# DRL-Navigation/DDRL4NAV

Hardware: AMD Instinct MI355X
Metric: env-steps/sec (whole node) + PPO update ms, Pong 256 envs at 1/2/4/8 GPUs (higher is better)
Workload: dtype f32 (f16x3 MFMA planes, fp32 accumulate)

## Files before the change

### ddrl4nav_amd/csrc/conv2.hip

```cpp
#include "engine2.h"

namespace ddrl {


using u4v = __attribute__((ext_vector_type(4))) unsigned;

constexpr int F1_PITCH = 168;
template <int NE>
struct Fwd1B {
  static constexpr int ROWS = 32 * NE, A_BYTES = 4 * NPL * 2 * ROWS * 16, PITCH = F1_PITCH, IMG_BYTES = 64 * PITCH;
  static constexpr int STAGE_BYTES = A_BYTES + IMG_BYTES, AQ = A_BYTES / 16, NAJ = AQ / 256;
  static constexpr size_t LDS_BYTES = 2 * STAGE_BYTES;
};

template <int NE, bool IND = false>
__global__ __launch_bounds__(256) void conv_fwd1_planes_kernel(const uint8_t* __restrict__ frames, const unsigned short* __restrict__ wp1b,
                                                               float* __restrict__ amax, const float* __restrict__ params, int64_t bias_off0,
                                                               int64_t bias_off1, float* __restrict__ out, int64_t out_es, int n,
                                                               unsigned* __restrict__ m1, int64_t m1_es, int C,
                                                               const int32_t* __restrict__ tab, int64_t n_planes) {
  using K = Fwd1B<NE>;
  extern __shared__ __attribute__((aligned(16))) char ldsb[];
  const int tid = threadIdx.x, lane = tid & 63, wc = tid >> 6, l31 = lane & 31, hi = lane >> 5;
  const int c0 = blockIdx.x * 256, ctot = n * C1_P, clast = min(c0 + 255, ctot - 1);
  const int b0 = c0 / 400, b1 = clast / 400, oyf0 = (c0 % 400) / 20, iy0_start = 4 * oyf0;
  int nrows0, nrows1 = 0;
  if (b1 == b0) {
    nrows0 = 4 * ((clast % 400) / 20 - oyf0) + 8;
  } else {
    nrows0 = 84 - iy0_start;
    nrows1 = 4 * ((clast % 400) / 20) + 8;
  }
  const int nd0 = nrows0 * 21, nd_total = nd0 + nrows1 * 21;
  const int64_t src0 = (int64_t)b0 * (C * 7056) + iy0_start * 84, src1 = (int64_t)b1 * (C * 7056);
  if (blockIdx.x == 0 && tid < (AMAX_DH - AMAX_FIRST_ACT) * 2) amax[amax_idx(AMAX_FIRST_ACT, 0) + tid] = 0.0f;
  int64_t imsrc[6];
  int imdst[6];
  int imoff[6];
  unsigned imsel = 0u;
#pragma unroll
  for (int j = 0; j < 6; ++j) {
    const int idx = tid + 256 * j;
    if constexpr (IND) {
      const bool second = idx < nd_total && idx >= nd0;
      imoff[j] = second ? (idx - nd0) * 4 : iy0_start * 84 + (idx < nd0 ? idx * 4 : 0);
      imsel |= (second ? 1u : 0u) << j;
    } else {
      imsrc[j] = (idx >= nd_total) ? src0 : (idx < nd0 ? src0 + idx * 4 : src1 + (idx - nd0) * 4);
    }
    imdst[j] = K::A_BYTES + (idx / 21) * K::PITCH + (idx % 21) * 8;
  }
  int abase[NE], bbase[2];
#pragma unroll
  for (int i = 0; i < NE; ++i) abase[i] = (hi * K::ROWS + i * 32 + l31) * 16;
#pragma unroll
  for (int j = 0; j < 2; ++j) {
    int c = c0 + wc * 64 + j * 32 + l31;
    if (c >= ctot) c = c0;
    const int b = c / 400, pix = c % 400, oy = pix / 20, ox = pix % 20;
    const int lr = (b == b0) ? (4 * oy - iy0_start) : (nrows0 + 4 * oy);
    bbase[j] = K::A_BYTES + (lr + hi) * K::PITCH + ox * 8;
  }
  unsigned imreg[4][6];
  if constexpr (IND) {
#pragma unroll
    for (int ch = 0; ch < 4; ++ch) {
      const int64_t pb0 = frame_plane_base(tab, b0, ch, n_planes), pb1 = frame_plane_base(tab, b1, ch, n_planes);
#pragma unroll
      for (int j = 0; j < 6; ++j) imreg[ch][j] = *(const unsigned*)(frames + (((imsel >> j) & 1u) ? pb1 : pb0) + imoff[j]);
    }
  } else {
#pragma unroll
    for (int ch = 0; ch < 4; ++ch)
#pragma unroll
      for (int j = 0; j < 6; ++j) imreg[ch][j] = *(const unsigned*)(frames + (ch < C ? ch : C - 1) * 7056 + imsrc[j]);
  }
  const int wave = wave_u();
  uint32_t woff[K::NAJ];
#pragma unroll
  for (int j = 0; j < K::NAJ; ++j) woff[j] = (uint32_t)((tid + 256 * j) * 16);
  auto stage_w = [&](int ch, char* st) {
    direct_copy((const char*)wp1b + (size_t)ch * K::A_BYTES, woff, (float*)st, wave, tid, K::AQ);
  };
  auto commit_img = [&](char* st, int ch) {
#pragma unroll
    for (int j = 0; j < 6; ++j) {
      if (tid + 256 * j < nd_total) {
        const unsigned v = imreg[ch][j];
        *(uint2*)(st + imdst[j]) = pixel_quad(v);
      }
    }
  };
  f32x16 acc[NE][2];
#pragma unroll
  for (int i = 0; i < NE; ++i)
#pragma unroll
    for (int j = 0; j < 2; ++j)
#pragma unroll
      for (int r = 0; r < 16; ++r) acc[i][j][r] = 0.0f;
  stage_w(0, ldsb);
  commit_img(ldsb, 0);
  wait_vmcnt<0>();
  __syncthreads();
#pragma unroll
  for (int ch = 0; ch < 4; ++ch) {
    if (ch >= C) break;
    const char* cur = ldsb + (ch & 1) * K::STAGE_BYTES;
    char* nxt = ldsb + ((ch + 1) & 1) * K::STAGE_BYTES;
    if (ch + 1 < C) stage_w(ch + 1, nxt);
#pragma unroll
    for (int g = 0; g < 4; ++g) {
      frag8 b[2];
#pragma unroll
      for (int j = 0; j < 2; ++j) {
        const uint2 lo = *(const uint2*)(cur + bbase[j] + g * (2 * K::PITCH));
        const uint2 hi4 = *(const uint2*)(cur + bbase[j] + g * (2 * K::PITCH) + 8);
        b[j] = __builtin_bit_cast(frag8, (u4v){lo.x, lo.y, hi4.x, hi4.y});
      }
#pragma unroll
      for (int p = NPL - 1; p >= 0; --p) {
        frag8 a[NE];
#pragma unroll
        for (int i = 0; i < NE; ++i) a[i] = *(const frag8*)(cur + abase[i] + ((g * NPL + p) * 2) * K::ROWS * 16);
#pragma unroll
        for (int i = 0; i < NE; ++i)
#pragma unroll
          for (int j = 0; j < 2; ++j) acc[i][j] = mfma_planes(a[i], b[j], acc[i][j]);
      }
    }
    if (ch + 1 < C) {
      commit_img(nxt, ch + 1);
      wait_vmcnt<0>();
    }
    __syncthreads();
  }
  float* bias = (float*)ldsb;
  if (tid < K::ROWS) bias[tid] = params[(tid >> 5 ? bias_off1 : bias_off0) + (tid & 31)];
  __syncthreads();
  float r255[NE];
#pragma unroll
  for (int i = 0; i < NE; ++i) r255[i] = 1.0f / (255.0f * plane_scale(amax[amax_idx(AMAX_W1, i)]));
#pragma unroll
  for (int j = 0; j < 2; ++j) {
    const int c = c0 + wc * 64 + j * 32 + l31;
    if (c >= ctot) continue;
    const int b = c / 400, pix = c % 400;
    const uint32_t lanep = (uint32_t)((b * A1_N + pix + hi * (4 * C1_P)) * 4);
#pragma unroll
    for (int i = 0; i < NE; ++i) {
      float* base = out + i * out_es;
      unsigned bits = 0u;
#pragma unroll
      for (int r = 0; r < 16; ++r) {
        const int oc = acc_row(r, hi);
        const float y = leaky_f(__builtin_fmaf(acc[i][j][r], r255[i], bias[i * 32 + oc]));
        st1_so(base + acc_row(r, 0) * C1_P, lanep, y);
        bits = __builtin_amdgcn_alignbit(bits, (unsigned)__builtin_elementwise_sub_sat((int)__float_as_uint(y), 1), 31);
      }
      if (m1 != nullptr) ((unsigned short*)(m1 + i * m1_es))[2 * (int64_t)c + hi] = (unsigned short)bits;
    }
  }
}

template <int NE>
struct Fwd1R {
  static constexpr int ROWS = 32 * NE, A_BYTES = 4 * NPL * 2 * ROWS * 16, PITCH = F1_PITCH, IMG_BYTES = 64 * PITCH;
  static constexpr int W_BYTES = 4 * A_BYTES, IMG_OFF = W_BYTES, GROUP_IMG = 4 * IMG_BYTES;
  static constexpr int BIAS_OFF = IMG_OFF + 2 * GROUP_IMG;
  static constexpr size_t LDS_BYTES = BIAS_OFF + ROWS * 4;
  static_assert(LDS_BYTES <= 160 * 1024, "one workgroup per CU");
};

template <int NE, bool IND = false>
__global__ __launch_bounds__(512) void conv_fwd1_resident_kernel(const uint8_t* __restrict__ frames, const unsigned short* __restrict__ wp1b,
                                                                 float* __restrict__ amax, const float* __restrict__ params, int64_t bias_off0,
                                                                 int64_t bias_off1, float* __restrict__ out, int64_t out_es, int n,
                                                                 unsigned* __restrict__ m1, int64_t m1_es, int C,
                                                                 const int32_t* __restrict__ tab, int64_t n_planes) {
  using K = Fwd1R<NE>;
  extern __shared__ __attribute__((aligned(16))) char ldsr[];
  const int tid = threadIdx.x, gq = tid >> 8, lt = tid & 255, lane = tid & 63, wc = (tid >> 6) & 3, l31 = lane & 31, hi = lane >> 5;
  char* img = ldsr + K::IMG_OFF + gq * K::GROUP_IMG;
  float* bias = (float*)(ldsr + K::BIAS_OFF);
  const int ctot = n * C1_P, ntiles = (ctot + 255) / 256;
  if (blockIdx.x == 0 && tid < (AMAX_DH - AMAX_FIRST_ACT) * 2) amax[amax_idx(AMAX_FIRST_ACT, 0) + tid] = 0.0f;
  for (int q = tid; q < C * (K::A_BYTES / 16); q += 512) *(f4*)(ldsr + q * 16) = *(const f4*)((const char*)wp1b + (size_t)q * 16);
  if (tid < K::ROWS) bias[tid] = params[(tid >> 5 ? bias_off1 : bias_off0) + (tid & 31)];
  float r255[NE];
#pragma unroll
  for (int i = 0; i < NE; ++i) r255[i] = 1.0f / (255.0f * plane_scale(amax[amax_idx(AMAX_W1, i)]));
  int abase[NE];
#pragma unroll
  for (int i = 0; i < NE; ++i) abase[i] = (hi * K::ROWS + i * 32 + l31) * 16;

  struct Geo {
    int c0, b0, iy0_start, nrows0, nd0, nd_total;
    int64_t src0, src1;
    int64_t pb[2][4];
  };
  auto geometry = [&](int t) {
    Geo g;
    g.c0 = t * 256;
    const int clast = min(g.c0 + 255, ctot - 1);
    g.b0 = g.c0 / 400;
    const int b1 = clast / 400, oyf0 = (g.c0 % 400) / 20;
    g.iy0_start = 4 * oyf0;
    int nrows1 = 0;
    if (b1 == g.b0) {
      g.nrows0 = 4 * ((clast % 400) / 20 - oyf0) + 8;
    } else {
      g.nrows0 = 84 - g.iy0_start;
      nrows1 = 4 * ((clast % 400) / 20) + 8;
    }
    g.nd0 = g.nrows0 * 21;
    g.nd_total = g.nd0 + nrows1 * 21;
    if constexpr (IND) {
      const int ub0 = __builtin_amdgcn_readfirstlane(g.b0), ub1 = __builtin_amdgcn_readfirstlane(b1);
#pragma unroll
      for (int ch = 0; ch < 4; ++ch) {
        g.pb[0][ch] = frame_plane_base(tab, ub0, ch, n_planes);
        g.pb[1][ch] = frame_plane_base(tab, ub1, ch, n_planes);
      }
      return g;
    }
    g.src0 = (int64_t)g.b0 * (C * 7056) + g.iy0_start * 84;
    g.src1 = (int64_t)b1 * (C * 7056);
    return g;
  };
  unsigned imreg[4][6];
  auto request = [&](const Geo& g) {
#pragma unroll
    for (int j = 0; j < 6; ++j) {
      const int idx = lt + 256 * j;
      if constexpr (IND) {
        const bool second = idx < g.nd_total && idx >= g.nd0;
        const int o = second ? (idx - g.nd0) * 4 : g.iy0_start * 84 + (idx < g.nd0 ? idx * 4 : 0);
#pragma unroll
        for (int ch = 0; ch < 4; ++ch) {
          const int64_t p0 = g.pb[0][ch], p1 = g.pb[1][ch];
          imreg[ch][j] = *(const unsigned*)(frames + (second ? p1 : p0) + o);
        }
        continue;
      }
      const int64_t o = (idx >= g.nd_total) ? g.src0 : (idx < g.nd0 ? g.src0 + idx * 4 : g.src1 + (idx - g.nd0) * 4);
#pragma unroll
      for (int ch = 0; ch < 4; ++ch) imreg[ch][j] = *(const unsigned*)(frames + (ch < C ? ch : C - 1) * 7056 + o);
    }
  };
  int t = 2 * (int)blockIdx.x + gq;
  Geo g = geometry(min(t, ntiles - 1));
  request(g);
  __syncthreads();
  for (; 2 * (t / 2) < ntiles; t += 2 * (int)gridDim.x) {
    const bool live = t < ntiles;
#pragma unroll
    for (int ch = 0; ch < 4; ++ch)
#pragma unroll
      for (int j = 0; j < 6; ++j) {
        const int idx = lt + 256 * j;
        if (ch < C && idx < g.nd_total) *(uint2*)(img + ch * K::IMG_BYTES + (idx / 21) * K::PITCH + (idx % 21) * 8) = pixel_quad(imreg[ch][j]);
      }
    int bbase[2];
#pragma unroll
    for (int j = 0; j < 2; ++j) {
      int c = g.c0 + wc * 64 + j * 32 + l31;
      if (c >= ctot) c = g.c0;
      const int b = c / 400, pix = c % 400, oy = pix / 20, ox = pix % 20;
      const int lr = (b == g.b0) ? (4 * oy - g.iy0_start) : (g.nrows0 + 4 * oy);
      bbase[j] = (lr + hi) * K::PITCH + ox * 8;
    }
    const Geo cur = g;
    __syncthreads();
    const int tn = t + 2 * (int)gridDim.x;
    if (2 * (tn / 2) < ntiles) {
      g = geometry(min(tn, ntiles - 1));
      request(g);
    }
    f32x16 acc[NE][2];
#pragma unroll
    for (int i = 0; i < NE; ++i)
#pragma unroll
      for (int j = 0; j < 2; ++j)
#pragma unroll
        for (int r = 0; r < 16; ++r) acc[i][j][r] = 0.0f;
#pragma unroll
    for (int ch = 0; ch < 4; ++ch) {
      if (ch >= C) break;
#pragma unroll
      for (int gk = 0; gk < 4; ++gk) {
        frag8 b[2];
#pragma unroll
        for (int j = 0; j < 2; ++j) {
          const char* q = img + ch * K::IMG_BYTES + bbase[j] + gk * (2 * K::PITCH);
          const uint2 lo = *(const uint2*)q, hi4 = *(const uint2*)(q + 8);
          b[j] = __builtin_bit_cast(frag8, (u4v){lo.x, lo.y, hi4.x, hi4.y});
        }
#pragma unroll
        for (int p = NPL - 1; p >= 0; --p) {
          frag8 a[NE];
#pragma unroll
          for (int i = 0; i < NE; ++i) a[i] = *(const frag8*)(ldsr + ch * K::A_BYTES + abase[i] + ((gk * NPL + p) * 2) * K::ROWS * 16);
#pragma unroll
          for (int i = 0; i < NE; ++i)
#pragma unroll
            for (int j = 0; j < 2; ++j) acc[i][j] = mfma_planes(a[i], b[j], acc[i][j]);
        }
      }
    }
    __syncthreads();
    if (!live) continue;
#pragma unroll
    for (int j = 0; j < 2; ++j) {
      const int c = cur.c0 + wc * 64 + j * 32 + l31;
      if (c >= ctot) continue;
      const int b = c / 400, pix = c % 400;
      const uint32_t lanep = (uint32_t)((b * A1_N + pix + hi * (4 * C1_P)) * 4);
#pragma unroll
      for (int i = 0; i < NE; ++i) {
        float* base = out + i * out_es;
        unsigned bits = 0u;
#pragma unroll
        for (int r = 0; r < 16; ++r) {
          const int oc = acc_row(r, hi);
          const float y = leaky_f(__builtin_fmaf(acc[i][j][r], r255[i], bias[i * 32 + oc]));
          st1_so(base + acc_row(r, 0) * C1_P, lanep, y);
          bits = __builtin_amdgcn_alignbit(bits, (unsigned)__builtin_elementwise_sub_sat((int)__float_as_uint(y), 1), 31);
        }
        if (m1 != nullptr) ((unsigned short*)(m1 + i * m1_es))[2 * (int64_t)c + hi] = (unsigned short)bits;
      }
    }
  }
}

template <int NE, bool IND>
static void launch_fwd1_planes(const EncCall& c, bool acting, hipStream_t st) {
  const Workspace& w = *c.ws;
  const ParamLayout& L = *c.L;
  if (!acting && (int64_t)c.n * C1_P >= 256 * 2048) {
    using R = Fwd1R<NE>;
    lds_limit_once<conv_fwd1_resident_kernel<NE, IND>>((int)R::LDS_BYTES);
    static const int cus = [] {
      int dev = 0;
      hipDeviceProp_t prop;
      return hipGetDevice(&dev) == hipSuccess && hipGetDeviceProperties(&prop, dev) == hipSuccess ? prop.multiProcessorCount : 256;
    }();
    hipLaunchKernelGGL((conv_fwd1_resident_kernel<NE, IND>), dim3((unsigned)cus), dim3(512), R::LDS_BYTES, st, c.frames, w.wp1b, w.amax, c.params,
                       L.enc_base[0] + L.enc.c1b, L.enc_base[NE - 1] + L.enc.c1b, w.a1, w.es(A1_N), c.n, w.m1, w.es(M1_N), L.C, c.tab, c.n_planes);
    return;
  }
  using K = Fwd1B<NE>;
  lds_limit_once<conv_fwd1_planes_kernel<NE, IND>>((int)K::LDS_BYTES);
  hipLaunchKernelGGL((conv_fwd1_planes_kernel<NE, IND>), dim3((unsigned)(((int64_t)c.n * C1_P + 255) / 256)), dim3(256), K::LDS_BYTES, st, c.frames,
                     w.wp1b, w.amax, c.params, L.enc_base[0] + L.enc.c1b, L.enc_base[NE - 1] + L.enc.c1b, w.a1, w.es(A1_N), c.n,
                     acting ? (unsigned*)nullptr : w.m1, w.es(M1_N), L.C, c.tab, c.n_planes);
}
template <int NE>
static void launch_fwd1(const EncCall& c, bool acting, hipStream_t st) {
  if (c.tab != nullptr) {
    launch_fwd1_planes<NE, true>(c, acting, st);
  } else {
    launch_fwd1_planes<NE, false>(c, acting, st);
  }
}

struct Fwd2B {
  static constexpr int SPT = 3, KC = 2;
  static constexpr int WPE = 3;
  static constexpr int ROW = 52, CH = 20 * ROW, IMG_PLANE = SPT * KC * CH;
  static constexpr int W_OFF = NPL * IMG_PLANE, W_BYTES = KC * NPL * 64 * 32;
  static constexpr int BIAS_OFF = W_OFF + W_BYTES;
  static constexpr int NIU = SPT * KC * 100, NIJ = (NIU + 255) / 256;
  static constexpr int NWJ = W_BYTES / 16 / 256;
  static constexpr int STAGE_BYTES = BIAS_OFF;
  static constexpr size_t LDS_BYTES = STAGE_BYTES + 64 * 4;
};
struct __attribute__((packed, aligned(4))) lds_u2 {
  unsigned x, y;
};

__global__ __launch_bounds__(256) __attribute__((amdgpu_waves_per_eu(Fwd2B::WPE, Fwd2B::WPE))) void conv_fwd2_planes_kernel(const float* __restrict__ a1, int64_t a1_es, const unsigned short* __restrict__ wp2b,
                                                               float* __restrict__ amax, const float* __restrict__ params, int64_t bias_off0,
                                                               int64_t bias_off1, float* __restrict__ out, int64_t out_es, int n,
                                                               unsigned* __restrict__ m2) {
  using K = Fwd2B;
  extern __shared__ __attribute__((aligned(16))) char ldsc2[];
  const int tid = threadIdx.x, lane = tid & 63, wc = tid >> 6, l31 = lane & 31, hi = lane >> 5;
  const int e = blockIdx.z, b0 = blockIdx.x * K::SPT;
  const float sa = plane_scale(amax[amax_idx(AMAX_A1, e)]), inv = 1.0f / (sa * plane_scale(amax[amax_idx(AMAX_W2, e)]));
  if (tid < 64) ((float*)(ldsc2 + K::STAGE_BYTES))[tid] = params[(e ? bias_off1 : bias_off0) + tid];
  const float* isrc[K::NIJ];
  int idst[K::NIJ];
#pragma unroll
  for (int j = 0; j < K::NIJ; ++j) {
    const int u = min(tid + 256 * j, K::NIU - 1);
    const int s = u / (100 * K::KC), rem = u % (100 * K::KC), q = rem % 100;
    isrc[j] = a1 + e * a1_es + (int64_t)min(b0 + s, n - 1) * A1_N + rem * 4;
    idst[j] = (s * K::KC + rem / 100) * K::CH + (q / 5) * K::ROW + (q % 5) * 8;
  }
  const unsigned short* wsrc = wp2b + (int64_t)e * (32 * NPL * 64 * 16) + tid * 8;
  int aA[2], bB[2];
#pragma unroll
  for (int i = 0; i < 2; ++i) aA[i] = K::W_OFF + (i * 32 + l31) * 32 + hi * 16;
#pragma unroll
  for (int j = 0; j < 2; ++j) {
    int c = wc * 64 + j * 32 + l31;
    if (c >= K::SPT * 81) c = 0;
    const int s = c / 81, pix = c % 81, oy = pix / 9, ox = pix % 9;
    bB[j] = s * K::KC * K::CH + (2 * oy + 2 * hi) * K::ROW + 4 * ox;
  }
  f4 ir[K::NIJ], wr[K::NWJ];
  auto fetch = [&](int kb) {
#pragma unroll
    for (int j = 0; j < K::NIJ; ++j) ir[j] = ld4(isrc[j] + kb * (C1_P * K::KC));
#pragma unroll
    for (int j = 0; j < K::NWJ; ++j) wr[j] = *(const f4*)(wsrc + kb * (K::KC * NPL * 1024) + j * 2048);
  };
  auto commit = [&](char* ldsc2) {
#pragma unroll
    for (int j = 0; j < K::NIJ; ++j) {
      if (j + 1 < K::NIJ || tid + 256 * j < K::NIU) {
        const f4 v = ir[j];
        unsigned pa[NPL], pb[NPL];
        split_planes(v.x, v.y, sa, pa);
        split_planes(v.z, v.w, sa, pb);
        char* d = ldsc2 + idst[j];
#pragma unroll
        for (int p = 0; p < NPL; ++p) *(lds_u2*)(d + p * K::IMG_PLANE) = lds_u2{pa[p], pb[p]};
      }
    }
#pragma unroll
    for (int j = 0; j < K::NWJ; ++j) *(f4*)(ldsc2 + K::W_OFF + (tid + 256 * j) * 16) = wr[j];
  };
  f32x16 acc[2][2];
#pragma unroll
  for (int i = 0; i < 2; ++i)
#pragma unroll
    for (int j = 0; j < 2; ++j)
#pragma unroll
      for (int r = 0; r < 16; ++r) acc[i][j][r] = 0.0f;
  constexpr int NKB = 32 / K::KC;
  auto compute = [&](const char* ldsc2) {
#pragma unroll
    for (int kg = 0; kg < K::KC; ++kg) {
      frag8 a[NPL][2], b[NPL][2];
#pragma unroll
      for (int p = 0; p < NPL; ++p) {
#pragma unroll
        for (int i = 0; i < 2; ++i) a[p][i] = *(const frag8*)(ldsc2 + aA[i] + (kg * NPL + p) * 2048);
#pragma unroll
        for (int j = 0; j < 2; ++j) {
          const char* q = ldsc2 + bB[j] + p * K::IMG_PLANE + kg * K::CH;
          const lds_u2 lo = *(const lds_u2*)q, up = *(const lds_u2*)(q + K::ROW);
          b[p][j] = __builtin_bit_cast(frag8, (u4v){lo.x, lo.y, up.x, up.y});
        }
      }
#pragma unroll
      for (int t = 0; t < NPROD; ++t)
#pragma unroll
        for (int i = 0; i < 2; ++i)
#pragma unroll
          for (int j = 0; j < 2; ++j) acc[i][j] = mfma_planes(a[PA[t]][i], b[PB[t]][j], acc[i][j]);
    }
  };
  fetch(0);
  commit(ldsc2);
  fetch(1);
  __syncthreads();
  for (int kb = 0; kb < NKB; ++kb) {
    compute(ldsc2);
    __syncthreads();
    if (kb + 1 < NKB) {
      commit(ldsc2);
      if (kb + 2 < NKB) fetch(kb + 2);
    }
    __syncthreads();
  }
  const float* bias = (const float*)(ldsc2 + K::STAGE_BYTES);
  float big = 0.0f;
#pragma unroll
  for (int j = 0; j < 2; ++j) {
    const int c = wc * 64 + j * 32 + l31;
    const int s = c / 81, pix = c % 81;
    if (c >= K::SPT * 81 || b0 + s >= n) continue;
    float* base = out + e * out_es + (int64_t)b0 * A2_N;
    const uint32_t lb = (uint32_t)((s * A2_N + pix + hi * (4 * C2_P)) * 4);
    unsigned bits = 0u;
#pragma unroll
    for (int i = 0; i < 2; ++i)
#pragma unroll
      for (int r = 0; r < 16; ++r) {
        const int oc = i * 32 + acc_row(r, hi);
        const float y = leaky_f(__builtin_fmaf(acc[i][j][r], inv, bias[oc]));
        st1_so(base + (i * 32 + acc_row(r, 0)) * C2_P, lb, y);
        big = fmaxf(big, fabsf(y));
        bits = __builtin_amdgcn_alignbit(bits, (unsigned)__builtin_elementwise_sub_sat((int)__float_as_uint(y), 1), 31);
      }
    if (m2 != nullptr) m2[(e * (out_es / A2_N) + b0 + s) * M2_N + pix * 2 + hi] = (bits >> 16) | (bits << 16);
  }
  amax_update(big, amax + amax_idx(AMAX_A2, e));
}
static void launch_fwd2_planes(const EncCall& c, bool acting, hipStream_t st) {
  using K = Fwd2B;
  const Workspace& w = *c.ws;
  const ParamLayout& L = *c.L;
  lds_limit_once<conv_fwd2_planes_kernel>((int)K::LDS_BYTES);
  hipLaunchKernelGGL(conv_fwd2_planes_kernel, dim3((unsigned)((c.n + K::SPT - 1) / K::SPT), 1, (unsigned)L.NE), dim3(256), K::LDS_BYTES, st, w.a1,
                     w.es(A1_N), w.wp2b, w.amax, c.params, L.enc_base[0] + L.enc.c2b, L.enc_base[L.NE - 1] + L.enc.c2b, w.a2, w.es(A2_N),
                     c.n, acting ? (unsigned*)nullptr : w.m2);
}

struct Fwd3B {
  static constexpr int WPE = 3;
  static constexpr int TN = 2, SPT = (128 * TN) / 49, NPX = SPT * 81;
  static constexpr int IMG_PLANE = NPX * 16;
  static constexpr int W_OFF = NPL * IMG_PLANE, W_BYTES = 5 * NPL * 64 * 32;
  static constexpr int BIAS_OFF = W_OFF + W_BYTES;
  static constexpr int NIJ = (NPX + 255) / 256;
  static constexpr int NWJ = (W_BYTES / 16 + 255) / 256;
  static constexpr size_t LDS_BYTES = BIAS_OFF + 64 * 4;
};

__global__ __launch_bounds__(256) __attribute__((amdgpu_waves_per_eu(Fwd3B::WPE, Fwd3B::WPE))) void conv_fwd3_planes_kernel(const float* __restrict__ a2, int64_t a2_es, const unsigned short* __restrict__ wp3b,
                                                               float* __restrict__ amax, const float* __restrict__ params, int64_t bias_off0,
                                                               int64_t bias_off1, float* __restrict__ out, int64_t out_es, int n,
                                                               unsigned* __restrict__ m3) {
  using K = Fwd3B;
  extern __shared__ __attribute__((aligned(16))) char ldsc3[];
  const int tid = threadIdx.x, lane = tid & 63, wc = tid >> 6, l31 = lane & 31, hi = lane >> 5;
  const int e = blockIdx.z, b0 = blockIdx.x * K::SPT;
  const float sa = plane_scale(amax[amax_idx(AMAX_A2, e)]), inv = 1.0f / (sa * plane_scale(amax[amax_idx(AMAX_W3, e)]));
  if (tid < 64) ((float*)(ldsc3 + K::BIAS_OFF))[tid] = params[(e ? bias_off1 : bias_off0) + tid];
  const float* isrc[K::NIJ];
#pragma unroll
  for (int j = 0; j < K::NIJ; ++j) {
    const int u = min(tid + 256 * j, K::NPX - 1);
    const int s = u / 81, px = u % 81;
    isrc[j] = a2 + e * a2_es + (int64_t)min(b0 + s, n - 1) * A2_N + px;
  }
  const unsigned short* wsrc = wp3b + (int64_t)e * (8 * 5 * NPL * 64 * 16) + tid * 8;
  int aA[2], bB[K::TN], tapoff[5];
#pragma unroll
  for (int i = 0; i < 2; ++i) aA[i] = K::W_OFF + (i * 32 + l31) * 32 + hi * 16;
#pragma unroll
  for (int j = 0; j < K::TN; ++j) {
    int c = wc * (32 * K::TN) + j * 32 + l31;
    if (c >= K::SPT * 49) c = 0;
    const int s = c / 49, pix = c % 49;
    bB[j] = (s * 81 + (pix / 7) * 9 + pix % 7) * 16;
  }
#pragma unroll
  for (int kg = 0; kg < 5; ++kg) {
    const int tap = min(2 * kg + hi, 8);
    tapoff[kg] = ((tap / 3) * 9 + tap % 3) * 16;
  }
  float ir[K::NIJ][8];
  f4 wr[K::NWJ];
  auto fetch = [&](int kb) {
#pragma unroll
    for (int j = 0; j < K::NIJ; ++j)
#pragma unroll
      for (int c = 0; c < 8; ++c) ir[j][c] = isrc[j][(kb * 8 + c) * C2_P];
#pragma unroll
    for (int j = 0; j < K::NWJ; ++j)
      if (j + 1 < K::NWJ || tid + 256 * j < K::W_BYTES / 16) wr[j] = *(const f4*)(wsrc + kb * (5 * NPL * 1024) + j * 2048);
  };
  auto commit = [&]() {
#pragma unroll
    for (int j = 0; j < K::NIJ; ++j) {
      if (j + 1 < K::NIJ || tid + 256 * j < K::NPX) {
        unsigned pl[4][NPL];
#pragma unroll
        for (int c = 0; c < 4; ++c) split_planes(ir[j][2 * c], ir[j][2 * c + 1], sa, pl[c]);
        char* d = ldsc3 + (tid + 256 * j) * 16;
#pragma unroll
        for (int p = 0; p < NPL; ++p) *(u4v*)(d + p * K::IMG_PLANE) = (u4v){pl[0][p], pl[1][p], pl[2][p], pl[3][p]};
      }
    }
#pragma unroll
    for (int j = 0; j < K::NWJ; ++j)
      if (j + 1 < K::NWJ || tid + 256 * j < K::W_BYTES / 16) *(f4*)(ldsc3 + K::W_OFF + (tid + 256 * j) * 16) = wr[j];
  };
  f32x16 acc[2][K::TN];
#pragma unroll
  for (int i = 0; i < 2; ++i)
#pragma unroll
    for (int j = 0; j < K::TN; ++j)
#pragma unroll
      for (int r = 0; r < 16; ++r) acc[i][j][r] = 0.0f;
  constexpr int NKB = 8;
  fetch(0);
  commit();
  fetch(1);
  __syncthreads();
  for (int kb = 0; kb < NKB; ++kb) {
#pragma unroll
    for (int kg = 0; kg < 5; ++kg) {
      frag8 a[NPL][2], b[NPL][K::TN];
#pragma unroll
      for (int p = 0; p < NPL; ++p) {
#pragma unroll
        for (int i = 0; i < 2; ++i) a[p][i] = *(const frag8*)(ldsc3 + aA[i] + (kg * NPL + p) * 2048);
#pragma unroll
        for (int j = 0; j < K::TN; ++j) b[p][j] = *(const frag8*)(ldsc3 + bB[j] + tapoff[kg] + p * K::IMG_PLANE);
      }
#pragma unroll
      for (int t = 0; t < NPROD; ++t)
#pragma unroll
        for (int i = 0; i < 2; ++i)
#pragma unroll
          for (int j = 0; j < K::TN; ++j) acc[i][j] = mfma_planes(a[PA[t]][i], b[PB[t]][j], acc[i][j]);
    }
    __syncthreads();
    if (kb + 1 < NKB) {
      commit();
      if (kb + 2 < NKB) fetch(kb + 2);
    }
    __syncthreads();
  }
  const float* bias = (const float*)(ldsc3 + K::BIAS_OFF);
  float big = 0.0f;
#pragma unroll
  for (int j = 0; j < K::TN; ++j) {
    const int c = wc * (32 * K::TN) + j * 32 + l31;
    const int s = c / 49, pix = c % 49;
    if (c >= K::SPT * 49 || b0 + s >= n) continue;
    float* base = out + e * out_es + (int64_t)b0 * FLAT;
    const uint32_t lb = (uint32_t)((s * A3_N + pix + hi * (4 * C3_P)) * 4);
    unsigned bits = 0u;
#pragma unroll
    for (int i = 0; i < 2; ++i)
#pragma unroll
      for (int r = 0; r < 16; ++r) {
        const int oc = i * 32 + acc_row(r, hi);
        const float y = leaky_f(__builtin_fmaf(acc[i][j][r], inv, bias[oc]));
        st1_so(base + (i * 32 + acc_row(r, 0)) * C3_P, lb, y);
        big = fmaxf(big, fabsf(y));
        bits = __builtin_amdgcn_alignbit(bits, (unsigned)__builtin_elementwise_sub_sat((int)__float_as_uint(y), 1), 31);
      }
    if (m3 != nullptr) m3[(e * (out_es / A3_N) + b0 + s) * M3_N + pix * 2 + hi] = (bits >> 16) | (bits << 16);
  }
  amax_update(big, amax + amax_idx(AMAX_A3, e));
}
static void launch_fwd3_planes(const EncCall& c, bool acting, hipStream_t st) {
  using K = Fwd3B;
  const Workspace& w = *c.ws;
  const ParamLayout& L = *c.L;
  lds_limit_once<conv_fwd3_planes_kernel>((int)K::LDS_BYTES);
  hipLaunchKernelGGL(conv_fwd3_planes_kernel, dim3((unsigned)((c.n + K::SPT - 1) / K::SPT), 1, (unsigned)L.NE), dim3(256), K::LDS_BYTES, st, w.a2,
                     w.es(A2_N), w.wp3b, w.amax, c.params, L.enc_base[0] + L.enc.c3b, L.enc_base[L.NE - 1] + L.enc.c3b, w.a3, w.es(A3_N),
                     c.n, acting ? (unsigned*)nullptr : w.m3);
}


void launch_conv_forward(const EncCall& c, bool acting, hipStream_t st) {
  {
    ProfRange pr(c.prof, acting ? "ConvFwd1.act" : "ConvFwd1", st);
    if (c.L->NE == 2) {
      launch_fwd1<2>(c, acting, st);
    } else {
      launch_fwd1<1>(c, acting, st);
    }
  }
  {
    ProfRange pr(c.prof, acting ? "ConvFwd2.act" : "ConvFwd2", st);
    launch_fwd2_planes(c, acting, st);
  }
  {
    ProfRange pr(c.prof, acting ? "ConvFwd3.act" : "ConvFwd3", st);
    launch_fwd3_planes(c, acting, st);
  }
}

struct Dgrad3Rows {
  static constexpr int SPT = 3, NCOL = SPT * 81, NT = 8, ROWW = SPT * 9;
  static constexpr int col_y(int c) { return c / ROWW; }
  static constexpr int col_s(int c) { return c % ROWW / 9; }
  static constexpr int col_x(int c) { return c % 9; }
  static constexpr int tile_y0(int t) { return col_y(32 * t); }
  static constexpr int tile_y1(int t) { return col_y(32 * t + 31 < NCOL ? 32 * t + 31 : NCOL - 1); }
  static constexpr bool tile_has_tap(int t, int tap) { return tap / 3 <= tile_y1(t) && tap / 3 + 6 >= tile_y0(t); }
  static constexpr int tile_taps(int t) {
    int m = 0;
    for (int tap = 0; tap < 9; ++tap) m |= (int)tile_has_tap(t, tap) << tap;
    return m;
  }
  static constexpr int WT = 3, NU = 4;
  static constexpr int WAVE_TILE[4][WT] = {{0, 1, -1}, {5, 6, -1}, {2, 3, 7}, {4, 3, 7}};
  static constexpr int UNIT_I[4][NU] = {{0, 1, 0, 1}, {0, 1, 0, 1}, {0, 1, 0, 0}, {0, 1, 1, 1}};
  static constexpr int UNIT_J[4][NU] = {{0, 0, 1, 1}, {0, 0, 1, 1}, {0, 0, 1, 2}, {0, 0, 1, 2}};
  static constexpr int unit_tile(int w, int u) { return WAVE_TILE[w][UNIT_J[w][u]]; }
  static constexpr int popcount9(int m) {
    int c = 0;
    for (int b = 0; b < 9; ++b) c += m >> b & 1;
    return c;
  }

  static constexpr bool tap_feeds_tile(int t, int tap) {
    for (int c = 32 * t; c < 32 * t + 32 && c < NCOL; ++c) {
      const int sy = col_y(c) - tap / 3, sx = col_x(c) - tap % 3;
      if (sy >= 0 && sy <= 6 && sx >= 0 && sx <= 6) return true;
    }
    return false;
  }
  static constexpr bool masks_are_exact() {
    for (int t = 0; t < NT; ++t)
      for (int tap = 0; tap < 9; ++tap)
        if (tap_feeds_tile(t, tap) != tile_has_tap(t, tap)) return false;
    return true;
  }
  static constexpr bool columns_are_a_permutation() {
    bool seen[NCOL] = {};
    for (int c = 0; c < NCOL; ++c) {
      const int k = col_s(c) * 81 + col_y(c) * 9 + col_x(c);
      if (col_s(c) >= SPT || col_y(c) >= 9 || seen[k]) return false;
      seen[k] = true;
    }
    return true;
  }
  static constexpr int owners(int i, int t) {
    int n = 0;
    for (int w = 0; w < 4; ++w)
      for (int u = 0; u < NU; ++u) n += UNIT_I[w][u] == i && UNIT_J[w][u] < WT && unit_tile(w, u) == t;
    return n;
  }
  static constexpr bool every_unit_has_one_owner() {
    for (int i = 0; i < 2; ++i)
      for (int t = 0; t < NT; ++t)
        if (owners(i, t) != 1) return false;
    return true;
  }
  static constexpr int wave_unit_taps(int w) {
    int n = 0;
    for (int u = 0; u < NU; ++u) n += popcount9(tile_taps(unit_tile(w, u)));
    return n;
  }
  static constexpr int row_tile_taps() {
    int n = 0;
    for (int t = 0; t < NT; ++t) n += popcount9(tile_taps(t));
    return n;
  }
};
static_assert(Dgrad3Rows::NT * 32 >= Dgrad3Rows::NCOL && (Dgrad3Rows::NT - 1) * 32 < Dgrad3Rows::NCOL, "8 column tiles of 32");
static_assert(Dgrad3Rows::columns_are_a_permutation(), "every (sample, pixel) is one column");
static_assert(Dgrad3Rows::masks_are_exact(), "a skipped (tile, tap) reads only the zero border, an issued one reads a dz3 pixel");
static_assert(Dgrad3Rows::every_unit_has_one_owner(), "each of the 16 accumulator tiles belongs to exactly one wave (four each)");
static_assert(Dgrad3Rows::row_tile_taps() == 60, "60 of 72 (column tile, tap) products per row tile");
static_assert(Dgrad3Rows::wave_unit_taps(0) == 30 && Dgrad3Rows::wave_unit_taps(1) == 30 && Dgrad3Rows::wave_unit_taps(2) == 30 &&
                  Dgrad3Rows::wave_unit_taps(3) == 30, "the waves are level: 30 unit-taps = 90 MFMAs per k-block each");

template <int V>
struct RoleC {
  static constexpr int value = V;
};
template <class F>
__device__ __forceinline__ void by_wave_role(int w, F&& f) {
  switch (w) {
    case 0: f(RoleC<0>{}); break;
    case 1: f(RoleC<1>{}); break;
    case 2: f(RoleC<2>{}); break;
    default: f(RoleC<3>{}); break;
  }
}

struct Dgrad3B {
  using R = Dgrad3Rows;
  static constexpr int THREADS = 256, SPT = R::SPT;
  static constexpr int KOC = 16, NKB = 64 / KOC, PIXB = 2 * KOC;
  static constexpr int IMG_PLANE = SPT * 121 * PIXB;
  static constexpr int W_OFF = NPL * IMG_PLANE, W_BYTES = 9 * NPL * 64 * 32;
  static constexpr int NIU = SPT * 49, NIJ = (NIU + THREADS - 1) / THREADS;
  static constexpr int NWQ = W_BYTES / 16, NWJ = (NWQ + THREADS - 1) / THREADS;
  static constexpr size_t LDS_BYTES = W_OFF + W_BYTES;
  static constexpr int OSS = 32 * C2_P + 16, OQS = 32 * C2_P / 4, NOJ = (SPT * OQS + THREADS - 1) / THREADS;
  static_assert(SPT * OSS * 4 <= (int)LDS_BYTES && (32 * C2_P) % 4 == 0 && OSS % 4 == 0 && A2_N % 4 == 0, "the staged half fits, 16-byte rows");
};

__global__ __launch_bounds__(Dgrad3B::THREADS) __attribute__((amdgpu_waves_per_eu(2, 2))) void conv_dgrad3_planes_kernel(
    const float* __restrict__ dz3, int64_t dz_es, const unsigned short* __restrict__ wd3b, float* __restrict__ amax, const unsigned* __restrict__ m2,
    float* __restrict__ out, int64_t out_es, int n) {
  using K = Dgrad3B;
  using R = K::R;
  extern __shared__ __attribute__((aligned(16))) char ldsd3[];
  const int tid = threadIdx.x, lane = tid & 63, wc = __builtin_amdgcn_readfirstlane(tid >> 6), l31 = lane & 31, hi = lane >> 5;
  const int e = blockIdx.z, b0 = blockIdx.x * K::SPT;
  const float sa = plane_scale(amax[amax_idx(AMAX_DZ3, e)]), inv = 1.0f / (sa * plane_scale(amax[amax_idx(AMAX_W3, e)]));
  for (int i = tid; i < K::W_OFF / 16; i += K::THREADS) *(f4*)(ldsd3 + i * 16) = zero4();
  const float* isrc[K::NIJ];
  int idst[K::NIJ];
#pragma unroll
  for (int j = 0; j < K::NIJ; ++j) {
    const int u = min(tid + K::THREADS * j, K::NIU - 1);
    const int s = u / 49, px = u % 49;
    isrc[j] = dz3 + e * dz_es + (int64_t)min(b0 + s, n - 1) * FLAT + px;
    idst[j] = (s * 121 + (px / 7 + 2) * 11 + px % 7 + 2) * K::PIXB;
  }
  const unsigned short* wsrc = wd3b + (int64_t)e * (K::NKB * 9 * NPL * 64 * 16) + tid * 8;
  int aA[2], bB[R::WT];
#pragma unroll
  for (int i = 0; i < 2; ++i) aA[i] = K::W_OFF + (i * 32 + l31) * 32 + hi * 16;
  by_wave_role(wc, [&](auto role) {
    constexpr int W = decltype(role)::value;
#pragma unroll
    for (int j = 0; j < R::WT; ++j) {
      int c = R::WAVE_TILE[W][j] * 32 + l31;
      if (R::WAVE_TILE[W][j] < 0 || c >= R::NCOL) c = 0;
      bB[j] = (R::col_s(c) * 121 + R::col_y(c) * 11 + R::col_x(c)) * K::PIXB + hi * 16;
    }
  });
  float ir[K::NIJ][K::KOC];
  f4 wr[K::NWJ];
  auto fetch = [&](int kb) {
#pragma unroll
    for (int j = 0; j < K::NIJ; ++j)
#pragma unroll
      for (int c = 0; c < K::KOC; ++c) ir[j][c] = isrc[j][(kb * K::KOC + c) * C3_P];
#pragma unroll
    for (int j = 0; j < K::NWJ; ++j)
      if (j + 1 < K::NWJ || tid + K::THREADS * j < K::NWQ) wr[j] = *(const f4*)(wsrc + kb * (9 * NPL * 1024) + j * (K::THREADS * 8));
  };
  auto commit = [&]() {
#pragma unroll
    for (int j = 0; j < K::NIJ; ++j) {
      if (j + 1 < K::NIJ || tid + K::THREADS * j < K::NIU) {
        unsigned pl[K::KOC / 2][NPL];
#pragma unroll
        for (int c = 0; c < K::KOC / 2; ++c) split_planes(ir[j][2 * c], ir[j][2 * c + 1], sa, pl[c]);
        char* d = ldsd3 + idst[j];
#pragma unroll
        for (int p = 0; p < NPL; ++p) {
          *(u4v*)(d + p * K::IMG_PLANE) = (u4v){pl[0][p], pl[1][p], pl[2][p], pl[3][p]};
          *(u4v*)(d + p * K::IMG_PLANE + 16) = (u4v){pl[4][p], pl[5][p], pl[6][p], pl[7][p]};
        }
      }
    }
#pragma unroll
    for (int j = 0; j < K::NWJ; ++j)
      if (j + 1 < K::NWJ || tid + K::THREADS * j < K::NWQ) *(f4*)(ldsd3 + K::W_OFF + (tid + K::THREADS * j) * 16) = wr[j];
  };
  f32x16 acc[R::NU];
#pragma unroll
  for (int u = 0; u < R::NU; ++u)
#pragma unroll
    for (int r = 0; r < 16; ++r) acc[u][r] = 0.0f;
  auto mma = [&](auto role) {
    constexpr int W = decltype(role)::value;
#pragma unroll
    for (int t = 0; t < 9; ++t) {
      constexpr int ROW11 = 11;
      const int toff = ((2 - t / 3) * ROW11 + 2 - t % 3) * K::PIXB;
      frag8 af[NPL][2], bfr[NPL][R::WT];
#pragma unroll
      for (int p = 0; p < NPL; ++p) {
#pragma unroll
        for (int i = 0; i < 2; ++i) af[p][i] = *(const frag8*)(ldsd3 + aA[i] + (t * NPL + p) * 2048);
#pragma unroll
        for (int j = 0; j < R::WT; ++j)
          if (R::WAVE_TILE[W][j] >= 0 && R::tile_has_tap(R::WAVE_TILE[W][j], t)) bfr[p][j] = *(const frag8*)(ldsd3 + bB[j] + toff + p * K::IMG_PLANE);
      }
#pragma unroll
      for (int m = 0; m < NPROD; ++m)
#pragma unroll
        for (int u = 0; u < R::NU; ++u)
          if (R::tile_has_tap(R::unit_tile(W, u), t)) acc[u] = mfma_planes(af[PA[m]][R::UNIT_I[W][u]], bfr[PB[m]][R::UNIT_J[W][u]], acc[u]);
    }
  };
  fetch(0);
  __syncthreads();
  commit();
  fetch(1);
  __syncthreads();
  by_wave_role(wc, [&](auto role) {
    for (int kb = 0; kb < K::NKB; ++kb) {
      mma(role);
      __syncthreads();
      if (kb + 1 < K::NKB) {
        commit();
        if (kb + 2 < K::NKB) fetch(kb + 2);
      }
      __syncthreads();
    }
  });
  float big = 0.0f;
  float* ob = (float*)ldsd3;
  unsigned mw[R::WT];
  int ocol[R::WT];
  by_wave_role(wc, [&](auto role) {
    constexpr int W = decltype(role)::value;
#pragma unroll
    for (int j = 0; j < R::WT; ++j) {
      const int c = R::WAVE_TILE[W][j] * 32 + l31;
      const int s = R::col_s(c), pix = R::col_y(c) * 9 + R::col_x(c);
      const bool live = R::WAVE_TILE[W][j] >= 0 && c < R::NCOL && b0 + s < n;
      ocol[j] = live ? s * K::OSS + hi * (4 * C2_P) + pix : -1;
      mw[j] = live ? m2[(e * (out_es / A2_N) + b0 + s) * M2_N + pix * 2 + hi] : 0u;
    }
  });
#pragma unroll
  for (int i = 0; i < 2; ++i) {
    if (i) __syncthreads();
    by_wave_role(wc, [&](auto role) {
      constexpr int W = decltype(role)::value;
#pragma unroll
      for (int u = 0; u < R::NU; ++u) {
        const int j = R::UNIT_J[W][u];
        if (R::UNIT_I[W][u] != i || ocol[j] < 0) continue;
#pragma unroll
        for (int r = 0; r < 16; ++r) {
          const float g = leaky_bit(mw[j], 16 * i + 15 - r, acc[u][r] * inv);
          ob[ocol[j] + acc_row(r, 0) * C2_P] = g;
          big = fmaxf(big, fabsf(g));
        }
      }
    });
    __syncthreads();
#pragma unroll
    for (int k = 0; k < K::NOJ; ++k) {
      const int q = tid + K::THREADS * k, s = q / K::OQS, w4 = q % K::OQS * 4;
      if (q < K::SPT * K::OQS && b0 + s < n) *(f4*)(out + e * out_es + (int64_t)(b0 + s) * A2_N + i * (32 * C2_P) + w4) = *(const f4*)(ob + s * K::OSS + w4);
    }
  }
  amax_update(big, amax + amax_idx(AMAX_DZ2, e));
}
static void launch_dgrad3_planes(const EncCall& c, hipStream_t st) {
  using K = Dgrad3B;
  const Workspace& w = *c.ws;
  lds_limit_once<conv_dgrad3_planes_kernel>((int)K::LDS_BYTES);
  hipLaunchKernelGGL(conv_dgrad3_planes_kernel, dim3((unsigned)((c.n + K::SPT - 1) / K::SPT), 1, (unsigned)c.L->NE), dim3(K::THREADS), K::LDS_BYTES, st,
                     w.dz3, w.es(A3_N), w.wd3b, w.amax, w.m2, w.dz2, w.es(A2_N), c.n);
}

void launch_conv_dgrad3(const EncCall& c, hipStream_t st) {
  ProfRange pr(c.prof, "ConvDgrad3", st);
  launch_dgrad3_planes(c, st);
}

struct Dgrad2Both {
  static constexpr int SPT = 5, THREADS = 512, TN = 2;
  static constexpr int IMG_PLANE = SPT * 121 * 16;
  static constexpr int W_HALF = 2 * NPL * 64 * 32;
  static constexpr int W_OFF = NPL * IMG_PLANE, W_BYTES = 2 * W_HALF;
  static constexpr int NIU = SPT * 81;
  static constexpr int NWQ = W_BYTES / 16, NWJ = NWQ / THREADS;
  static constexpr size_t LDS_BYTES = W_OFF + W_BYTES;
};

__global__ __launch_bounds__(512) __attribute__((amdgpu_waves_per_eu(2, 2))) void conv_dgrad2_both_kernel(
    const float* __restrict__ dz2, int64_t dz_es, const unsigned short* __restrict__ wd2b, float* __restrict__ amax, float* __restrict__ out,
    int64_t out_es, int n) {
  using K = Dgrad2Both;
  extern __shared__ __attribute__((aligned(16))) char ldsd2[];
  const int tid = threadIdx.x, lane = tid & 63, wc = tid >> 6, l31 = lane & 31, hi = lane >> 5;
  const int e = blockIdx.y, b0 = blockIdx.x * K::SPT;
  const float sa = plane_scale(amax[amax_idx(AMAX_DZ2, e)]), inv = 1.0f / (sa * plane_scale(amax[amax_idx(AMAX_W2, e)]));
  for (int i = tid; i < K::W_OFF / 16; i += K::THREADS) *(f4*)(ldsd2 + i * 16) = zero4();
  const int u = min(tid, K::NIU - 1);
  const float* isrc = dz2 + e * dz_es + (int64_t)min(b0 + u / C2_P, n - 1) * A2_N + u % C2_P;
  const int idst = ((u / 81) * 121 + ((u % 81) / 9 + 1) * 11 + (u % 81) % 9 + 1) * 16;
  const unsigned short* wsrc[K::NWJ];
#pragma unroll
  for (int j = 0; j < K::NWJ; ++j) {
    const int q = tid + K::THREADS * j, par = q / (K::W_HALF / 16), qh = q % (K::W_HALF / 16);
    wsrc[j] = wd2b + (int64_t)(e * 2 + par) * (8 * 2 * NPL * 64 * 16) + qh * 8;
  }
  int aA[4], bB[K::TN];
#pragma unroll
  for (int i = 0; i < 4; ++i) aA[i] = K::W_OFF + (i >> 1) * K::W_HALF + ((i & 1) * 32 + l31) * 32 + hi * 16;
#pragma unroll
  for (int j = 0; j < K::TN; ++j) {
    int c = wc * (32 * K::TN) + j * 32 + l31;
    if (c >= K::SPT * 100) c = 0;
    const int s = c / 100, pq = c % 100;
    bB[j] = (s * 121 + (pq / 10 + 1) * 11 + (pq % 10 + 1) - hi) * 16;
  }
  float ir[8];
  f4 wr[K::NWJ];
  auto fetch = [&](int kb) {
#pragma unroll
    for (int c = 0; c < 8; ++c) ir[c] = isrc[(kb * 8 + c) * C2_P];
#pragma unroll
    for (int j = 0; j < K::NWJ; ++j) wr[j] = *(const f4*)(wsrc[j] + kb * (2 * NPL * 1024));
  };
  auto commit = [&]() {
    if (tid < K::NIU) {
      unsigned pl[4][NPL];
#pragma unroll
      for (int c = 0; c < 4; ++c) split_planes(ir[2 * c], ir[2 * c + 1], sa, pl[c]);
      char* d = ldsd2 + idst;
#pragma unroll
      for (int p = 0; p < NPL; ++p) *(u4v*)(d + p * K::IMG_PLANE) = (u4v){pl[0][p], pl[1][p], pl[2][p], pl[3][p]};
    }
#pragma unroll
    for (int j = 0; j < K::NWJ; ++j) *(f4*)(ldsd2 + K::W_OFF + (tid + K::THREADS * j) * 16) = wr[j];
  };
  f32x16 acc[4][K::TN];
#pragma unroll
  for (int i = 0; i < 4; ++i)
#pragma unroll
    for (int j = 0; j < K::TN; ++j)
#pragma unroll
      for (int r = 0; r < 16; ++r) acc[i][j][r] = 0.0f;
  constexpr int NKB = 8;
  fetch(0);
  __syncthreads();
  commit();
  fetch(1);
  __syncthreads();
  for (int kb = 0; kb < NKB; ++kb) {
#pragma unroll
    for (int kg = 0; kg < 2; ++kg) {
      frag8 af[NPL][4], bfr[NPL][K::TN];
#pragma unroll
      for (int p = 0; p < NPL; ++p) {
#pragma unroll
        for (int i = 0; i < 4; ++i) af[p][i] = *(const frag8*)(ldsd2 + aA[i] + (kg * NPL + p) * 2048);
#pragma unroll
        for (int j = 0; j < K::TN; ++j) bfr[p][j] = *(const frag8*)(ldsd2 + bB[j] + p * K::IMG_PLANE - kg * (11 * 16));
      }
#pragma unroll
      for (int t = 0; t < NPROD; ++t)
#pragma unroll
        for (int i = 0; i < 4; ++i)
#pragma unroll
          for (int j = 0; j < K::TN; ++j) acc[i][j] = mfma_planes(af[PA[t]][i], bfr[PB[t]][j], acc[i][j]);
    }
    __syncthreads();
    if (kb + 1 < NKB) {
      commit();
      if (kb + 2 < NKB) fetch(kb + 2);
    }
    __syncthreads();
  }
  float big = 0.0f;
#pragma unroll
  for (int j = 0; j < K::TN; ++j) {
    const int c = wc * (32 * K::TN) + j * 32 + l31;
    const int s = c / 100, pq = c % 100;
    if (c >= K::SPT * 100 || b0 + s >= n) continue;
#pragma unroll
    for (int a = 0; a < 2; ++a) {
      float* base = out + e * out_es + (int64_t)(b0 + s) * A1_N + (2 * (pq / 10) + a) * 20 + 2 * (pq % 10);
#pragma unroll
      for (int r = 0; r < 16; ++r) {
        const float g0 = acc[2 * a][j][r] * inv, g1 = acc[2 * a + 1][j][r] * inv;
        *(float2*)(base + acc_row(r, hi) * C1_P) = make_float2(g0, g1);
        big = fmaxf(big, fmaxf(fabsf(g0), fabsf(g1)));
      }
    }
  }
  amax_update(big, amax + amax_idx(AMAX_DZ1, e));
}

void launch_conv_dgrad2(const EncCall& c, hipStream_t st) {
  const Workspace& w = *c.ws;
  ProfRange pr(c.prof, "ConvDgrad2", st);
  lds_limit_once<conv_dgrad2_both_kernel>((int)Dgrad2Both::LDS_BYTES);
  hipLaunchKernelGGL(conv_dgrad2_both_kernel, dim3((unsigned)((c.n + Dgrad2Both::SPT - 1) / Dgrad2Both::SPT), (unsigned)c.L->NE, 1),
                     dim3(Dgrad2Both::THREADS), Dgrad2Both::LDS_BYTES, st, w.dz2, w.es(A2_N), w.wd2b, w.amax, w.dz1, w.es(A1_N), c.n);
}

}
```

Measured before the change: 260,200.

## Restructure fwd3 conv into 16-channel k-blocks with two tap sub-stages

The conv3 forward kernel now stages 16 input channels per k-block instead of 8. Each k-block runs as two tap sub-stages (5 taps, then 4) that share one weight buffer, and the weight gather no longer loads the zero padding tap. The aim is fewer k-block iterations and barriers per channel, no wasted padding-tap weight traffic, and LDS kept within the budget for three workgroups per CU. In exchange the kernel carries more image registers, a more complex fetch/commit schedule with extra syncs per k-block, and depends on constexpr-checked weight indexing.

```diff
diff --git a/ddrl4nav_amd/csrc/conv2.hip b/ddrl4nav_amd/csrc/conv2.hip
--- a/ddrl4nav_amd/csrc/conv2.hip
+++ b/ddrl4nav_amd/csrc/conv2.hip
@@ -511,14 +511,55 @@
 
 struct Fwd3B {
   static constexpr int WPE = 3;
+  static constexpr int TAPS_A = 5;
   static constexpr int TN = 2, SPT = (128 * TN) / 49, NPX = SPT * 81;
-  static constexpr int IMG_PLANE = NPX * 16;
-  static constexpr int W_OFF = NPL * IMG_PLANE, W_BYTES = 5 * NPL * 64 * 32;
+  static constexpr int KCH = 16, NKB = 64 / KCH;
+  static constexpr int IMG_OCT = NPX * 16, IMG_PLANE = 2 * IMG_OCT;
+  static constexpr int TAPS_B = 9 - TAPS_A;
+  static constexpr int SLAB = 2 * 64 * 16, SLAB_Q = SLAB / 16;
+  static constexpr int W_OFF = NPL * IMG_PLANE, W_BYTES = TAPS_A * NPL * SLAB;
   static constexpr int BIAS_OFF = W_OFF + W_BYTES;
   static constexpr int NIJ = (NPX + 255) / 256;
-  static constexpr int NWJ = (W_BYTES / 16 + 255) / 256;
+  static constexpr int NWJ = (TAPS_A * NPL * SLAB_Q + 255) / 256;
   static constexpr size_t LDS_BYTES = BIAS_OFF + 64 * 4;
+  static constexpr int tap_off(int tap) { return ((tap / 3) * 9 + tap % 3) * 16; }
+  static constexpr int WP3B_QUADS = 8 * 5 * NPL * 64 * 2;
+  static constexpr int wp3b_quad(int kb, int tap, int oct, int p, int oc) {
+    return ((((2 * kb + oct) * 5 + tap / 2) * NPL + p) * 64 + oc) * 2 + tap % 2;
+  }
+  static constexpr bool is_zero_quad(int q) { return q / (NPL * 64 * 2) % 5 == 4 && q % 2 == 1; }
+  static constexpr bool gather_is_exact() {
+    unsigned char hits[WP3B_QUADS] = {};
+    for (int kb = 0; kb < NKB; ++kb)
+      for (int tap = 0; tap < 9; ++tap)
+        for (int oct = 0; oct < 2; ++oct)
+          for (int p = 0; p < NPL; ++p)
+            for (int oc = 0; oc < 64; ++oc) {
+              const int q = wp3b_quad(kb, tap, oct, p, oc);
+              if (q < 0 || q >= WP3B_QUADS || hits[q]) return false;
+              hits[q] = 1;
+            }
+    int nonzero = 0;
+    for (int q = 0; q < WP3B_QUADS; ++q) {
+      if (hits[q] == is_zero_quad(q)) return false;
+      nonzero += hits[q];
+    }
+    return nonzero == NPL * 64 * 9 * 8;
+  }
+  static constexpr bool gather_is_separable() {
+    for (int kb = 0; kb < NKB; ++kb)
+      for (int tap = 0; tap < 9; ++tap)
+        for (int oct = 0; oct < 2; ++oct)
+          for (int p = 0; p < NPL; ++p)
+            for (int oc = 0; oc < 64; ++oc)
+              if (wp3b_quad(kb, tap, oct, p, oc) != wp3b_quad(kb, tap, 0, p, 0) + wp3b_quad(0, 0, oct, 0, oc)) return false;
+    return true;
+  }
 };
+static_assert(Fwd3B::gather_is_exact(), "the gather copies each of the NPL x 64 x 9 x 8 non-zero quads of wp3b once and no quad of the zero tap");
+static_assert(Fwd3B::gather_is_separable(), "quad = uniform part (k-block, tap, plane) + lane part (octet, oc)");
+static_assert(Fwd3B::NKB * Fwd3B::KCH == 64 && Fwd3B::TAPS_B <= Fwd3B::TAPS_A, "four k-blocks of 16 channels; sub-stage two fits the buffer of sub-stage one");
+static_assert(Fwd3B::LDS_BYTES <= 54272, "three workgroups share a CU's 160 KB (106 allocation units of 512 B each)");
 
 __global__ __launch_bounds__(256) __attribute__((amdgpu_waves_per_eu(Fwd3B::WPE, Fwd3B::WPE))) void conv_fwd3_planes_kernel(const float* __restrict__ a2, int64_t a2_es, const unsigned short* __restrict__ wp3b,
                                                                float* __restrict__ amax, const float* __restrict__ params, int64_t bias_off0,
@@ -537,48 +578,57 @@
     const int s = u / 81, px = u % 81;
     isrc[j] = a2 + e * a2_es + (int64_t)min(b0 + s, n - 1) * A2_N + px;
   }
-  const unsigned short* wsrc = wp3b + (int64_t)e * (8 * 5 * NPL * 64 * 16) + tid * 8;
-  int aA[2], bB[K::TN], tapoff[5];
-#pragma unroll
-  for (int i = 0; i < 2; ++i) aA[i] = K::W_OFF + (i * 32 + l31) * 32 + hi * 16;
+  static_assert(256 % K::SLAB_Q == 0, "a wave's quads of one j lie in one slab");
+  constexpr int SPJ = 256 / K::SLAB_Q;
+  static_assert(SPJ == 2, "256 threads, 128 quads per slab");
+  const int wslab = __builtin_amdgcn_readfirstlane(tid / K::SLAB_Q) & 1;
+  const unsigned short* wsrc = wp3b + (int64_t)e * (K::WP3B_QUADS * 8) + K::wp3b_quad(0, 0, (tid >> 6) & 1, 0, tid & 63) * 8;
+  int aA[2], bB[K::TN];
+#pragma unroll
+  for (int i = 0; i < 2; ++i) aA[i] = K::W_OFF + hi * (64 * 16) + (i * 32 + l31) * 16;
 #pragma unroll
   for (int j = 0; j < K::TN; ++j) {
     int c = wc * (32 * K::TN) + j * 32 + l31;
     if (c >= K::SPT * 49) c = 0;
     const int s = c / 49, pix = c % 49;
-    bB[j] = (s * 81 + (pix / 7) * 9 + pix % 7) * 16;
-  }
-#pragma unroll
-  for (int kg = 0; kg < 5; ++kg) {
-    const int tap = min(2 * kg + hi, 8);
-    tapoff[kg] = ((tap / 3) * 9 + tap % 3) * 16;
-  }
-  float ir[K::NIJ][8];
+    bB[j] = hi * K::IMG_OCT + (s * 81 + (pix / 7) * 9 + pix % 7) * 16;
+  }
+  float ir[K::NIJ][K::KCH];
   f4 wr[K::NWJ];
-  auto fetch = [&](int kb) {
+  auto fetch_img = [&](int kb) {
 #pragma unroll
     for (int j = 0; j < K::NIJ; ++j)
 #pragma unroll
-      for (int c = 0; c < 8; ++c) ir[j][c] = isrc[j][(kb * 8 + c) * C2_P];
-#pragma unroll
-    for (int j = 0; j < K::NWJ; ++j)
-      if (j + 1 < K::NWJ || tid + 256 * j < K::W_BYTES / 16) wr[j] = *(const f4*)(wsrc + kb * (5 * NPL * 1024) + j * 2048);
-  };
-  auto commit = [&]() {
+      for (int c = 0; c < K::KCH; ++c) ir[j][c] = isrc[j][(kb * K::KCH + c) * C2_P];
+  };
+  auto commit_img = [&]() {
 #pragma unroll
     for (int j = 0; j < K::NIJ; ++j) {
       if (j + 1 < K::NIJ || tid + 256 * j < K::NPX) {
-        unsigned pl[4][NPL];
-#pragma unroll
-        for (int c = 0; c < 4; ++c) split_planes(ir[j][2 * c], ir[j][2 * c + 1], sa, pl[c]);
+        unsigned pl[K::KCH / 2][NPL];
+#pragma unroll
+        for (int c = 0; c < K::KCH / 2; ++c) split_planes(ir[j][2 * c], ir[j][2 * c + 1], sa, pl[c]);
         char* d = ldsc3 + (tid + 256 * j) * 16;
 #pragma unroll
-        for (int p = 0; p < NPL; ++p) *(u4v*)(d + p * K::IMG_PLANE) = (u4v){pl[0][p], pl[1][p], pl[2][p], pl[3][p]};
-      }
-    }
+        for (int p = 0; p < NPL; ++p)
+#pragma unroll
+          for (int o = 0; o < 2; ++o)
+            *(u4v*)(d + p * K::IMG_PLANE + o * K::IMG_OCT) = (u4v){pl[4 * o][p], pl[4 * o + 1][p], pl[4 * o + 2][p], pl[4 * o + 3][p]};
+      }
+    }
+  };
+  auto has_slab = [&](int j, int nt) { return SPJ * j < nt * NPL && (SPJ * j + SPJ <= nt * NPL || wslab + SPJ * j < nt * NPL); };
+  auto fetch_w = [&](int kb, int t0, int nt) {
+#pragma unroll
+    for (int j = 0; j < K::NWJ; ++j) {
+      const int slab = wslab + SPJ * j;
+      if (has_slab(j, nt)) wr[j] = *(const f4*)(wsrc + K::wp3b_quad(kb, t0 + slab / NPL, 0, slab % NPL, 0) * 8);
+    }
+  };
+  auto commit_w = [&](int nt) {
 #pragma unroll
     for (int j = 0; j < K::NWJ; ++j)
-      if (j + 1 < K::NWJ || tid + 256 * j < K::W_BYTES / 16) *(f4*)(ldsc3 + K::W_OFF + (tid + 256 * j) * 16) = wr[j];
+      if (has_slab(j, nt)) *(f4*)(ldsc3 + K::W_OFF + (tid + 256 * j) * 16) = wr[j];
   };
   f32x16 acc[2][K::TN];
 #pragma unroll
@@ -587,34 +637,47 @@
     for (int j = 0; j < K::TN; ++j)
 #pragma unroll
       for (int r = 0; r < 16; ++r) acc[i][j][r] = 0.0f;
-  constexpr int NKB = 8;
-  fetch(0);
-  commit();
-  fetch(1);
+  auto compute = [&](int t0, int nt) {
+#pragma unroll
+    for (int t = 0; t < K::TAPS_A; ++t) {
+      if (t >= nt) break;
+      frag8 a[NPL][2], b[NPL][K::TN];
+#pragma unroll
+      for (int p = 0; p < NPL; ++p) {
+#pragma unroll
+        for (int i = 0; i < 2; ++i) a[p][i] = *(const frag8*)(ldsc3 + aA[i] + (t * NPL + p) * K::SLAB);
+#pragma unroll
+        for (int j = 0; j < K::TN; ++j) b[p][j] = *(const frag8*)(ldsc3 + bB[j] + K::tap_off(t0 + t) + p * K::IMG_PLANE);
+      }
+#pragma unroll
+      for (int m = 0; m < NPROD; ++m)
+#pragma unroll
+        for (int i = 0; i < 2; ++i)
+#pragma unroll
+          for (int j = 0; j < K::TN; ++j) acc[i][j] = mfma_planes(a[PA[m]][i], b[PB[m]][j], acc[i][j]);
+    }
+  };
+  fetch_img(0);
+  fetch_w(0, 0, K::TAPS_A);
+  commit_img();
+  commit_w(K::TAPS_A);
+  fetch_w(0, K::TAPS_A, K::TAPS_B);
   __syncthreads();
-  for (int kb = 0; kb < NKB; ++kb) {
-#pragma unroll
-    for (int kg = 0; kg < 5; ++kg) {
-      frag8 a[NPL][2], b[NPL][K::TN];
-#pragma unroll
-      for (int p = 0; p < NPL; ++p) {
-#pragma unroll
-        for (int i = 0; i < 2; ++i) a[p][i] = *(const frag8*)(ldsc3 + aA[i] + (kg * NPL + p) * 2048);
-#pragma unroll
-        for (int j = 0; j < K::TN; ++j) b[p][j] = *(const frag8*)(ldsc3 + bB[j] + tapoff[kg] + p * K::IMG_PLANE);
-      }
-#pragma unroll
-      for (int t = 0; t < NPROD; ++t)
-#pragma unroll
-        for (int i = 0; i < 2; ++i)
-#pragma unroll
-          for (int j = 0; j < K::TN; ++j) acc[i][j] = mfma_planes(a[PA[t]][i], b[PB[t]][j], acc[i][j]);
-    }
+  for (int kb = 0; kb < K::NKB; ++kb) {
+    compute(0, K::TAPS_A);
     __syncthreads();
-    if (kb + 1 < NKB) {
-      commit();
-      if (kb + 2 < NKB) fetch(kb + 2);
-    }
+    commit_w(K::TAPS_B);
+    if (kb + 1 < K::NKB) {
+      fetch_img(kb + 1);
+      fetch_w(kb + 1, 0, K::TAPS_A);
+    }
+    __syncthreads();
+    compute(K::TAPS_A, K::TAPS_B);
+    if (kb + 1 == K::NKB) break;
+    __syncthreads();
+    commit_img();
+    commit_w(K::TAPS_A);
+    fetch_w(kb + 1, K::TAPS_A, K::TAPS_B);
     __syncthreads();
   }
   const float* bias = (const float*)(ldsc3 + K::BIAS_OFF);
```

Measured after the change: 261,100 (median of 6 runs). Within noise of the previous version (+0.4%).
